# torchkge-team/torchkge

Measured on AMD Instinct MI355X. Metric: link-prediction triples scored/sec (filtered LP eval, both sides), higher is better.
Workload: dtype f32 (f16 hi/lo-split MFMA prefilter + exact f32 recheck; ranks bit-identical to f32)

## Files before the change

### torchkge_amd/csrc/kge_common.h

```cpp
#pragma once
#include <hip/hip_runtime.h>
#include <stdint.h>
#include <stdlib.h>
#include "../../include/kge_hip.h"

#define KGE_WAVE 64

#define KGE_CHECK_LAUNCH()                          \
    do {                                            \
        hipError_t e__ = hipGetLastError();         \
        if (e__ != hipSuccess) return (int)e__;     \
    } while (0)

static inline hipStream_t kge_s(kge_stream_t s) { return reinterpret_cast<hipStream_t>(s); }

int kge_bilinear_score_fwd(int kind, const float *t0, const float *t1, int d_ent, int d_rel, const int64_t *h,
                           const int64_t *t, const int64_t *r, int64_t B, float *out, hipStream_t s);
int kge_bilinear_score_bwd(int kind, const float *t0, const float *t1, int d_ent, int d_rel, const int64_t *h,
                           const int64_t *t, const int64_t *r, int64_t B, const float *go, float *g0, float *g1,
                           float *rows, int64_t rows_ld, hipStream_t s);

int kge_transr_score_fwd(const float *E, const float *R, const float *M, int d_ent, int d_rel, const int64_t *h,
                         const int64_t *t, const int64_t *r, int64_t B, float *out, hipStream_t s);
int kge_transr_score_bwd(const float *E, const float *R, const float *M, int d_ent, int d_rel, const int64_t *h,
                         const int64_t *t, const int64_t *r, int64_t B, const float *go, float *rows, int64_t rows_ld,
                         hipStream_t s);

static inline bool kge_aligned16(const void *p) { return (reinterpret_cast<uintptr_t>(p) & 15) == 0; }

__device__ __forceinline__ void kge_atomic_max_u32(unsigned *addr, unsigned v)
{
    if (v > __builtin_nontemporal_load(addr)) atomicMax(addr, v);
}

__device__ __forceinline__ float wave_sum(float v)
{
#pragma unroll
    for (int o = 32; o > 0; o >>= 1) v += __shfl_xor(v, o, 64);
    return v;
}
__device__ __forceinline__ int wave_sum_i(int v)
{
#pragma unroll
    for (int o = 32; o > 0; o >>= 1) v += __shfl_xor(v, o, 64);
    return v;
}

__device__ __forceinline__ float lp_chain_dot(const float *__restrict__ a, const float *__restrict__ t,
                                              int K, float acc)
{
    int kb = 0;
    for (; kb + 8 <= K; kb += 8) {
        float av[8], tv[8];
#pragma unroll
        for (int j = 0; j < 8; ++j) { av[j] = a[kb + j]; tv[j] = t[kb + j]; }
#pragma unroll
        for (int j = 0; j < 4; ++j) {
            acc = fmaf(av[j], tv[j], acc);
            acc = fmaf(av[4 + j], tv[4 + j], acc);
        }
    }
    if (kb < K) {
#pragma unroll
        for (int j = 0; j < 4; ++j) {
            const int k0 = kb + j, k1 = kb + 4 + j;
            if (k0 < K) acc = fmaf(a[k0], t[k0], acc);
            if (k1 < K) acc = fmaf(a[k1], t[k1], acc);
        }
    }
    return acc;
}

__device__ __forceinline__ float lp_epilogue(int mode, float dot, float qn, float en)
{
    if (mode == KGE_LP_L2_EXPAND) {
        float d2 = fmaf(-2.0f, dot, qn + en);
        return -fmaxf(d2, 0.0f);
    }
    return dot;
}

__device__ __forceinline__ float lp_epilogue_proj(int mode, float v0, float x, float y, float p, float z)
{
    float v;
    if (mode == KGE_LP_L2_PROJH) v = fmaf(x, fmaf(x, z, p), v0);
    else v = fmaf(y, fmaf(y, z, fmaf(2.0f, x, p)), v0);
    return -fmaxf(v, 0.0f);
}
__device__ __forceinline__ float lp_epilogue_any(const kge_lp_desc &d, float dot, int64_t i, int64_t c)
{
    if (d.mode == KGE_LP_DOT) return dot;
    const float v0 = fmaf(-2.0f, dot, d.qn[i] + d.en[c]);
    if (d.mode == KGE_LP_L2_EXPAND) return -fmaxf(v0, 0.0f);
    const float x = d.scal[d.r_idx[i] * d.scal_ld + c];
    const float y = d.mode == KGE_LP_L2_PROJD ? d.yc[c] : 0.f;
    return lp_epilogue_proj(d.mode, v0, x, y, d.Wq[i * d.ldw], d.Wq[i * d.ldw + 1]);
}

constexpr float KGE_TWO_PI_F = 6.2831855f;
template <int MODE>
__device__ __forceinline__ float lp_direct_term(float x)
{
    if (MODE == KGE_LP_TORUS_L1) {
        const float a = fabsf(x);
        return fminf(a, 1.0f - a);
    } else if (MODE == KGE_LP_TORUS_L2) {
        const float v = x * x;
        return fminf(v, 1.0f - v);
    } else if (MODE == KGE_LP_TORUS_EL2) {
        const float u = fminf(x, 1.0f - x);
        return 1.0f - cosf(KGE_TWO_PI_F * u);
    }
    return fabsf(x);
}
template <int MODE>
__device__ __forceinline__ float lp_direct_finish(float acc)
{
    if (MODE == KGE_LP_TORUS_L1) return -(2.0f * acc);
    if (MODE == KGE_LP_TORUS_L2) return -(4.0f * acc);
    if (MODE == KGE_LP_TORUS_EL2) return -(0.5f * acc);
    return -acc;
}
template <int MODE>
__device__ __forceinline__ float lp_group_chain(const float *q, const float *t, int K)
{
    float acc = 0.0f;
    for (int k = 0; k < K; k += 4) {
        float m[4];
#pragma unroll
        for (int e = 0; e < 4; ++e) m[e] = lp_direct_term<MODE>(k + e < K ? q[k + e] - t[k + e] : 0.0f);
        acc = acc + ((m[0] + m[1]) + (m[2] + m[3]));
    }
    return acc;
}

__device__ __forceinline__ float lp_pair_score(const kge_lp_desc &d, int64_t i, int64_t c)
{
    if (KGE_LP_IS_MFMA(d.mode)) {
        float acc = lp_chain_dot(d.A0 + i * d.lda0, d.T0 + c * d.ldt0, d.K0, 0.0f);
        if (d.K1 > 0) acc = lp_chain_dot(d.A1 + i * d.lda1, d.T1 + c * d.ldt1, d.K1, acc);
        return lp_epilogue_any(d, acc, i, c);
    }
    const float *q = d.A0 + i * d.lda0;
    const float *t = d.T0 + c * d.ldt0;
    switch (d.mode) {
    case KGE_LP_TORUS_L1: return lp_direct_finish<KGE_LP_TORUS_L1>(lp_group_chain<KGE_LP_TORUS_L1>(q, t, d.K0));
    case KGE_LP_TORUS_L2: return lp_direct_finish<KGE_LP_TORUS_L2>(lp_group_chain<KGE_LP_TORUS_L2>(q, t, d.K0));
    case KGE_LP_TORUS_EL2: return lp_direct_finish<KGE_LP_TORUS_EL2>(lp_group_chain<KGE_LP_TORUS_EL2>(q, t, d.K0));
    default: break;
    }
    float acc = 0.0f;
    const bool l1 = d.mode == KGE_LP_L1_DIRECT;
    const float a = d.Wq ? d.scal[c * d.scal_ld + (d.scal_ld > 1 ? d.r_idx[i] : 0)] : 0.0f;
    const float *w = d.Wq ? d.Wq + i * d.ldw : nullptr;
    if (l1) {
        for (int k = 0; k < d.K0; k += 4) {
            float m[4];
#pragma unroll
            for (int e = 0; e < 4; ++e) {
                float diff = 0.0f;
                if (k + e < d.K0) {
                    diff = q[k + e] - t[k + e];
                    if (w) diff = fmaf(a, w[k + e], diff);
                }
                m[e] = fabsf(diff);
            }
            acc = acc + ((m[0] + m[1]) + (m[2] + m[3]));
        }
    } else {
        for (int k = 0; k < d.K0; ++k) {
            float diff = q[k] - t[k];
            if (w) diff = fmaf(a, w[k], diff);
            acc = fmaf(diff, diff, acc);
        }
    }
    return -acc;
}

#ifndef KGE_PS_KC_V
#define KGE_PS_KC_V 32
#define KGE_PS_LD_V 36
#endif
constexpr int KGE_PS_KC = KGE_PS_KC_V, KGE_PS_LD = KGE_PS_LD_V;

static inline bool kge_lp_vec4(const kge_lp_desc &d)
{
    bool v = (d.K0 % 4 == 0) && (d.lda0 % 4 == 0) && (d.ldt0 % 4 == 0) && kge_aligned16(d.A0) && kge_aligned16(d.T0);
    if (d.K1 > 0)
        v = v && (d.K1 % 4 == 0) && (d.lda1 % 4 == 0) && (d.ldt1 % 4 == 0) && kge_aligned16(d.A1) && kge_aligned16(d.T1);
    return v;
}

template <int CH>
__device__ __forceinline__ float lp_chain_direct(const float *__restrict__ a, const float *__restrict__ t, int K, float acc)
{
    if (CH != 2) {
        constexpr int OP = CH == 1 ? (int)KGE_LP_L1_DIRECT : CH;
        for (int k = 0; k < K; k += 4) {
            const float4 av = *reinterpret_cast<const float4 *>(a + k), tv = *reinterpret_cast<const float4 *>(t + k);
            acc = acc + ((lp_direct_term<OP>(av.x - tv.x) + lp_direct_term<OP>(av.y - tv.y)) +
                         (lp_direct_term<OP>(av.z - tv.z) + lp_direct_term<OP>(av.w - tv.w)));
        }
    } else {
        for (int k = 0; k < K; ++k) {
            const float diff = a[k] - t[k];
            acc = fmaf(diff, diff, acc);
        }
    }
    return acc;
}

template <bool VEC4, int CH = 0>
__device__ __forceinline__ float lp_staged_segment(const float *__restrict__ A, int64_t lda,
                                                   const float *__restrict__ T, int64_t ldt, int K, int qi, int ci,
                                                   float *qs, float *es, float acc)
{
    const int lane = threadIdx.x & 63;
    static_assert(KGE_PS_KC == 32, "the fetch / store macros below are written out for 8 float4 pieces per row");
    int k0 = 0;
    if (VEC4 && K >= KGE_PS_KC) {
        float4 q0, q1, q2, q3, q4, q5, q6, q7, e0, e1, e2, e3, e4, e5, e6, e7;
#define KGE_PS_FETCH(IT, KK)                                                                                  \
    {                                                                                                         \
        const int idx_ = lane + 64 * IT, rr_ = idx_ >> 3, pc_ = idx_ & 7;                                     \
        const int rq_ = __shfl(qi, rr_, 64), rc_ = __shfl(ci, rr_, 64);                                      \
        q##IT = *reinterpret_cast<const float4 *>(A + (int64_t)rq_ * lda + (KK) + pc_ * 4);                   \
        e##IT = *reinterpret_cast<const float4 *>(T + (int64_t)rc_ * ldt + (KK) + pc_ * 4);                   \
    }
#define KGE_PS_STORE(IT)                                                                                      \
    {                                                                                                         \
        const int idx_ = lane + 64 * IT, rr_ = idx_ >> 3, pc_ = idx_ & 7;                                     \
        *reinterpret_cast<float4 *>(qs + rr_ * KGE_PS_LD + pc_ * 4) = q##IT;                                  \
        *reinterpret_cast<float4 *>(es + rr_ * KGE_PS_LD + pc_ * 4) = e##IT;                                  \
    }
#define KGE_PS_ALL(M, ...) M(0, ##__VA_ARGS__) M(1, ##__VA_ARGS__) M(2, ##__VA_ARGS__) M(3, ##__VA_ARGS__) \
                           M(4, ##__VA_ARGS__) M(5, ##__VA_ARGS__) M(6, ##__VA_ARGS__) M(7, ##__VA_ARGS__)
        KGE_PS_ALL(KGE_PS_FETCH, 0)
        for (; k0 + KGE_PS_KC <= K; k0 += KGE_PS_KC) {
            KGE_PS_ALL(KGE_PS_STORE)
            if (k0 + 2 * KGE_PS_KC <= K) { KGE_PS_ALL(KGE_PS_FETCH, k0 + KGE_PS_KC) }
            __builtin_amdgcn_fence(__ATOMIC_SEQ_CST, "wavefront");
            if (CH == 0) acc = lp_chain_dot(qs + lane * KGE_PS_LD, es + lane * KGE_PS_LD, KGE_PS_KC, acc);
            else acc = lp_chain_direct<CH>(qs + lane * KGE_PS_LD, es + lane * KGE_PS_LD, KGE_PS_KC, acc);
            __builtin_amdgcn_fence(__ATOMIC_SEQ_CST, "wavefront");
        }
#undef KGE_PS_ALL
#undef KGE_PS_STORE
#undef KGE_PS_FETCH
    }
// ... 120 lines not shown
```

### torchkge_amd/csrc/lp_split_mfma.hip

```cpp
#include "kge_common.h"
#ifndef KGE_BUILD_NO_SLP
#error "build with -fno-slp-vectorize -DKGE_BUILD_NO_SLP=1 (torchkge_amd/csrc/build.py): SLP-packed v_pk_fma_f32 with a lane-crossing op_sel misreads beside co-executing MFMAs (profiles/r06/slp_bisect.txt)"
#endif

typedef _Float16 f16x8 __attribute__((ext_vector_type(8)));
typedef float f32x2 __attribute__((ext_vector_type(2)));
typedef float f32x16 __attribute__((ext_vector_type(16)));

namespace {

constexpr int TQ = 192, TC = 256;
constexpr int NT = 3;
constexpr int E_STAGE_BYTES = TC * 128;
constexpr int Q_STAGE_BYTES = TQ * 128;
constexpr int STAGE_BYTES = E_STAGE_BYTES + Q_STAGE_BYTES;
constexpr int UNC_CAP = 2048;
constexpr int GSETS = 4;
constexpr int SMEM_BYTES = 2 * STAGE_BYTES + 16 + UNC_CAP * 4 + TQ * 20 + TQ * GSETS * 12 + 16;
constexpr int SPLIT_SCALE_LOG2 = 12;

struct SplitParams {
    const char *Es, *Qs;
    int row_bytes;
    int units;
// ... 1861 lines not shown
                            *p.overflow = 1.0f;
                        }
                    }
                    if (lane == 0) *unc_cnt = 0;
                }
            }
            if (GS && more && !(dbg & 16)) {
                if (LV == 1) { KGE_HLOAD(ah0, bh0, sb_next, 0) } else { KGE_SLOAD(ah0, al0, bh0, bl0, sb_next, 0) }
            }
            if (more) {
                int qp_next, ct_next;
                item_qp_ct(it + 1, qp_next, ct_next);
                const int64_t next_q0 = (int64_t)qp_next * TQ;
                if (next_q0 != cur_q0) {
                    flush_counts(cur_q0);
                    cur_q0 = next_q0;
                    load_panel(cur_q0);
                }
            }
        }
        if (DBG && tl) {
            tsv[15] = __builtin_readcyclecounter();
            if (lane == 0) {
                unsigned long long *o = reinterpret_cast<unsigned long long *>(p.list) + ((wid >> 2) * KGE_TL_STAGES + g) * 16;
#pragma unroll
                for (int i = 0; i < 16; ++i) o[i] = tsv[i];
            }
        }
        if (++s == S) { s = 0; ++it; }
    }
#undef KGE_TS
#undef KGE_SMMA_PA
#undef KGE_SMMA_P
#undef KGE_HLOAD
#undef KGE_HWAIT
#undef KGE_SLOAD
#undef KGE_SWAIT
#undef KGE_DSR
    flush_counts(cur_q0);
}

template <bool VEC4>
__global__ __launch_bounds__(64, 2) void split_recheck_kernel(const kge_lp_desc d, const float *__restrict__ s_true,
                                                           const int32_t *__restrict__ list, int32_t cap,
                                                           const int32_t *__restrict__ list_count, int32_t *raw_count,
                                                           float *list_stat)
{
    __shared__ __attribute__((aligned(16))) float qs[64 * KGE_PS_LD];
    __shared__ __attribute__((aligned(16))) float es[64 * KGE_PS_LD];
    const int lane = threadIdx.x;
    const int n = (int)min((unsigned)*list_count, (unsigned)cap);
    if (list_stat && blockIdx.x == 0 && lane == 0) atomicAdd(list_stat, (float)n);
    const int ngroups = (n + 63) >> 6;
    for (int grp = blockIdx.x; grp < ngroups; grp += gridDim.x) {
        const int pi = grp * 64 + lane;
        const bool valid = pi < n;
        const int pj = valid ? pi : grp * 64;
        const int qi = list[2 * pj], ci = list[2 * pj + 1];
        const float sc = lp_pair_score_staged<VEC4>(d, qi, ci, qs, es);
        if (valid && !(sc >= s_true[qi])) atomicSub(&raw_count[qi], 1);
    }
}

__device__ __forceinline__ float recheck_e_segment(const float *__restrict__ T, int64_t ldt, int K, int ci,
                                                   const float *__restrict__ qrow, float *es, float acc)
{
    const int lane = threadIdx.x & 63;
    int k0 = 0;
    if (K >= KGE_PS_KC) {
        float4 e0, e1, e2, e3, e4, e5, e6, e7;
#define KGE_RR_FETCH(IT, KK)                                                                                  \
    {                                                                                                         \
        const int idx_ = lane + 64 * IT, rr_ = idx_ >> 3, pc_ = idx_ & 7;                                     \
        const int rc_ = __shfl(ci, rr_, 64);                                                                  \
        e##IT = *reinterpret_cast<const float4 *>(T + (int64_t)rc_ * ldt + (KK) + pc_ * 4);                   \
    }
#define KGE_RR_STORE(IT)                                                                                      \
    {                                                                                                         \
        const int idx_ = lane + 64 * IT, rr_ = idx_ >> 3, pc_ = idx_ & 7;                                     \
        *reinterpret_cast<float4 *>(es + rr_ * KGE_PS_LD + pc_ * 4) = e##IT;                                  \
    }
#define KGE_RR_ALL(M, ...) M(0, ##__VA_ARGS__) M(1, ##__VA_ARGS__) M(2, ##__VA_ARGS__) M(3, ##__VA_ARGS__) \
                           M(4, ##__VA_ARGS__) M(5, ##__VA_ARGS__) M(6, ##__VA_ARGS__) M(7, ##__VA_ARGS__)
        KGE_RR_ALL(KGE_RR_FETCH, 0)
        for (; k0 + KGE_PS_KC <= K; k0 += KGE_PS_KC) {
            KGE_RR_ALL(KGE_RR_STORE)
            if (k0 + 2 * KGE_PS_KC <= K) { KGE_RR_ALL(KGE_RR_FETCH, k0 + KGE_PS_KC) }
            __builtin_amdgcn_fence(__ATOMIC_SEQ_CST, "wavefront");
            acc = lp_chain_dot(qrow + k0, es + lane * KGE_PS_LD, KGE_PS_KC, acc);
            __builtin_amdgcn_fence(__ATOMIC_SEQ_CST, "wavefront");
        }
#undef KGE_RR_ALL
#undef KGE_RR_STORE
#undef KGE_RR_FETCH
    }
    for (; k0 < K; k0 += KGE_PS_KC) {
        const int kc = min(KGE_PS_KC, K - k0);
        const int pieces = kc >> 2;
        for (int idx = lane; idx < 64 * pieces; idx += 64) {
            const int rr = idx / pieces, pc = idx - rr * pieces;
            const int rc = __shfl(ci, rr, 64);
            *reinterpret_cast<float4 *>(es + rr * KGE_PS_LD + pc * 4) =
                *reinterpret_cast<const float4 *>(T + (int64_t)rc * ldt + k0 + pc * 4);
        }
        __builtin_amdgcn_fence(__ATOMIC_SEQ_CST, "wavefront");
        acc = lp_chain_dot(qrow + k0, es + lane * KGE_PS_LD, kc, acc);
        __builtin_amdgcn_fence(__ATOMIC_SEQ_CST, "wavefront");
    }
    return acc;
}

constexpr int RR_ROWS = 32, RR_PANEL = 96;

constexpr int RR_G = 4;

template <int NWV>
__global__ __launch_bounds__(64 * NWV) void split_recheck_regions_kernel(const kge_lp_desc d, const float *__restrict__ s_true,
                                                                        const int32_t *__restrict__ list, int32_t region_cap,
                                                                        const int32_t *__restrict__ region_count, int n_regions,
                                                                        int ldq, int seg_cols, int32_t *raw_count, float *list_stat,
                                                                        int32_t *list_count)
{
    extern __shared__ __attribute__((aligned(16))) float rr_smem[];
    const int tid = threadIdx.x, lane = tid & 63, wv = tid >> 6;
    float *qrows = rr_smem;
    float *es = rr_smem + RR_ROWS * ldq + wv * 64 * KGE_PS_LD;
    const int K = d.K0 + d.K1;
    int n_block = 0;
    auto stage = [&](int64_t q0, int c0, int c1) {
        const int np = (c1 - c0) >> 2;
        for (int idx = tid; idx < RR_ROWS * np; idx += 64 * NWV) {
            const int rr = idx / np, pc = idx - rr * np;
            const int64_t q = min(q0 + rr, d.B - 1);
            const int col = c0 + pc * 4;
            const float4 v = col < d.K0 ? *reinterpret_cast<const float4 *>(d.A0 + q * d.lda0 + col)
                                        : *reinterpret_cast<const float4 *>(d.A1 + q * d.lda1 + (col - d.K0));
            *reinterpret_cast<float4 *>(qrows + rr * ldq + pc * 4) = v;
        }
    };
    auto chain = [&](float acc, int ci, const float *qrow, int c0, int c1) -> float {
        if (c0 < d.K0) acc = recheck_e_segment(d.T0 + c0, d.ldt0, min(c1, d.K0) - c0, ci, qrow, es, acc);
        if (c1 > d.K0 && d.K1 > 0) {
            const int s0 = max(c0, d.K0);
            acc = recheck_e_segment(d.T1 + (s0 - d.K0), d.ldt1, c1 - s0, ci, qrow + (s0 - c0), es, acc);
        }
        return acc;
    };
    for (int reg = blockIdx.x; reg < n_regions; reg += gridDim.x) {
        const int n = (int)min((unsigned)region_count[reg], (unsigned)region_cap);
        if (n == 0) continue;
        n_block += n;
        const int64_t q0 = (int64_t)(reg / 3) * RR_PANEL + (reg % 3) * RR_ROWS;
        const int2 *ent = reinterpret_cast<const int2 *>(list) + (int64_t)reg * region_cap;
        if (K <= seg_cols) {
            __syncthreads();
            stage(q0, 0, K);
            __syncthreads();
            for (int c0 = wv * 64; c0 < n; c0 += NWV * 64) {
                const int pi = c0 + lane;
                const bool valid = pi < n;
                const int2 e = ent[valid ? pi : c0];
                const int qi = e.x, ci = e.y;
                const float acc = chain(0.0f, ci, qrows + (int)(qi - q0) * ldq, 0, K);
                const float sc = lp_epilogue_any(d, acc, qi, ci);
                if (valid && !(sc >= s_true[qi])) atomicSub(&raw_count[qi], 1);
            }
            continue;
        }
        for (int b0 = 0; b0 < n; b0 += NWV * 64 * RR_G) {
            float acc[RR_G];
            int qi[RR_G], ci[RR_G];
#pragma unroll
            for (int g = 0; g < RR_G; ++g) {
                const int c0 = b0 + (g * NWV + wv) * 64;
                const int pi = c0 + lane;
                const int2 e = ent[min(pi < n ? pi : c0, n - 1)];
                qi[g] = e.x; ci[g] = e.y; acc[g] = 0.0f;
            }
            for (int c0 = 0; c0 < K; c0 += seg_cols) {
                const int c1 = min(K, c0 + seg_cols);
                __syncthreads();
                stage(q0, c0, c1);
                __syncthreads();
#pragma unroll
                for (int g = 0; g < RR_G; ++g)
                    if (b0 + (g * NWV + wv) * 64 < n)
                        acc[g] = chain(acc[g], ci[g], qrows + (int)(qi[g] - q0) * ldq, c0, c1);
            }
#pragma unroll
            for (int g = 0; g < RR_G; ++g) {
                const int pi = b0 + (g * NWV + wv) * 64 + lane;
                if (pi < n) {
                    const float sc = lp_epilogue_any(d, acc[g], qi[g], ci[g]);
                    if (!(sc >= s_true[qi[g]])) atomicSub(&raw_count[qi[g]], 1);
                }
            }
        }
    }
    if (tid == 0 && n_block > 0) {
        if (list_stat) atomicAdd(list_stat, (float)n_block);
        if (list_count) atomicAdd(list_count, n_block);
    }
}

template <int NWAVES, bool DBG, int PM, int GS = 0, int LV = 0>
int launch_split(const SplitParams &p, int grid, hipStream_t s)
{
    auto k = lp_split_count_kernel<NWAVES, DBG, PM, GS, LV>;
    static int attr_dev[16];
    if (int e = kge_ensure_dyn_smem(reinterpret_cast<const void *>(k), SMEM_BYTES, attr_dev)) return e;
    hipLaunchKernelGGL(k, dim3(grid), dim3(64 * NWAVES), SMEM_BYTES, s, p);
    KGE_CHECK_LAUNCH();
    return 0;
}

int split_num_cus()
{
    static int n = 0;
    if (n == 0) {
        int dev = 0;
        hipDeviceProp_t prop;
        if (hipGetDevice(&dev) == hipSuccess && hipGetDeviceProperties(&prop, dev) == hipSuccess)
            n = prop.multiProcessorCount;
        if (n <= 0) n = 256;
    }
    return n;
}

inline int64_t round_up(int64_t x, int64_t m) { return (x + m - 1) / m * m; }

}

extern "C" int kge_lp_split_units(int K, int with_aug)
{
    return (int)round_up((K + (with_aug ? 1 : 0) + 15) / 16, 2);
}

extern "C" int64_t kge_lp_split_rows_padded(int64_t rows, int is_query) { return round_up(rows, is_query ? TQ : TC); }

extern "C" int kge_lp_split_rows(const float *X0, int64_t ld0, int K0, const float *X1, int64_t ld1, int K1,
                                 int64_t rows, int is_query, int aug_mode, const float *aug, float aug_mul,
                                 const float *norm2max0, const float *norm2max1, void *out, float *cell_ss,
                                 const int64_t *row_index, kge_stream_t stream)
{
    if (rows < 0 || K0 <= 0 || K1 < 0 || ld0 < K0 || (K1 > 0 && ld1 < K1) || aug_mode < 0 || aug_mode > 4)
        return KGE_EINVAL;
    if (rows == 0 && is_query) return 0;
    if ((rows > 0 && !X0) || (rows > 0 && K1 > 0 && !X1) || !out || ((aug_mode == 1 || aug_mode == 3) && rows > 0 && !aug))
        return KGE_EINVAL;
    SplitRowsParams p;
    p.X0 = X0; p.X1 = X1; p.ld0 = ld0; p.ld1 = ld1; p.K0 = K0; p.K1 = K1;
    p.rows = rows;
    p.rows_p = kge_lp_split_rows_padded(rows, is_query);
    p.aug_mode = aug_mode; p.aug = aug; p.aug_mul = aug_mul;
    p.nmax0 = norm2max0; p.nmax1 = norm2max1;
    p.units_p = kge_lp_split_units(K0 + K1, aug_mode != 0);
    p.out = reinterpret_cast<uint4 *>(out);
    p.cell_ss = cell_ss;
    p.row_index = row_index;
    const int64_t total = (p.rows_p / 16) * ((p.units_p + 15) / 16);
    if (total == 0) return 0;
    const int grid = (int)(total < 65536 ? total : 65536);
    hipLaunchKernelGGL(split_rows_kernel, dim3(grid), dim3(256), 0, kge_s(stream), p);
    KGE_CHECK_LAUNCH();
    return 0;
}

extern "C" int kge_lp_hi_units(int K) { return (int)round_up((K + 2 + 15) / 16, 4); }

static int hi_rows_impl(const float *X0, int64_t ld0, int K0, const float *X1, int64_t ld1, int K1, int64_t rows,
                        int is_query, int aug_mode, const float *aug, float aug_mul, const float *norm2max0,
                        const float *norm2max1, void *out, float *dn2, float *dn2max, const int64_t *row_index,
                        int frag, kge_stream_t stream)
{
    if (rows < 0 || K0 <= 0 || K1 < 0 || ld0 < K0 || (K1 > 0 && ld1 < K1) || aug_mode < 1 || aug_mode > 4) return KGE_EINVAL;
    if (rows == 0 && is_query) return 0;
    if ((rows > 0 && !X0) || (rows > 0 && K1 > 0 && !X1) || !out || ((aug_mode == 1 || aug_mode == 3) && rows > 0 && !aug))
        return KGE_EINVAL;
    HiRowsParams p;
    p.X0 = X0; p.X1 = X1; p.ld0 = ld0; p.ld1 = ld1; p.K0 = K0; p.K1 = K1;
    p.rows = rows;
    p.rows_p = kge_lp_split_rows_padded(rows, is_query);
    p.aug_mode = aug_mode; p.aug = aug; p.aug_mul = aug_mul;
    p.nmax0 = norm2max0; p.nmax1 = norm2max1;
    p.units_p = kge_lp_hi_units(K0 + K1);
    p.out = reinterpret_cast<uint4 *>(out);
    p.dn2 = dn2; p.dn2max = dn2max; p.row_index = row_index;
    p.frag = frag;
    p.nm_bmax = nullptr; p.nm_blocks = 0; p.dn_bmax = nullptr; p.prev_nmax = nullptr; p.nm_out = nullptr;
    const int64_t blocks = p.rows_p / 16;
    if (blocks == 0) return 0;
    const int64_t cap = dn2max ? 2 * (int64_t)split_num_cus() : 65536;
    hipLaunchKernelGGL(hi_rows_kernel, dim3((int)(blocks < cap ? blocks : cap)), dim3(256), 0, kge_s(stream), p);
    KGE_CHECK_LAUNCH();
    return 0;
}

extern "C" int kge_lp_hi_rows(const float *X0, int64_t ld0, int K0, const float *X1, int64_t ld1, int K1, int64_t rows,
                              int is_query, int aug_mode, const float *aug, float aug_mul, const float *norm2max0,
                              const float *norm2max1, void *out, float *dn2, float *dn2max, const int64_t *row_index,
                              kge_stream_t stream)
{
    return hi_rows_impl(X0, ld0, K0, X1, ld1, K1, rows, is_query, aug_mode, aug, aug_mul, norm2max0, norm2max1, out, dn2,
                        dn2max, row_index, 0, stream);
}

extern "C" int kge_lp_hi_rows_frag(const float *X0, int64_t ld0, int K0, const float *X1, int64_t ld1, int K1, int64_t rows,
                                   int aug_mode, const float *aug, float aug_mul, const float *norm2max0,
                                   const float *norm2max1, void *out, float *dn2, float *dn2max, kge_stream_t stream)
{
    return hi_rows_impl(X0, ld0, K0, X1, ld1, K1, rows, 0, aug_mode, aug, aug_mul, norm2max0, norm2max1, out, dn2, dn2max,
                        nullptr, 1, stream);
}

extern "C" int kge_lp_dot_table_prep_blocks(int64_t rows, int which)
{
    if (which == 0) { const int64_t b = (rows + 63) / 64; return (int)(b < 2048 ? (b > 0 ? b : 1) : 2048); }
    const int64_t b = kge_lp_split_rows_padded(rows, 0) / 16;
    return (int)(b < 4096 ? (b > 0 ? b : 1) : 4096);
}

extern "C" int kge_lp_dot_table_prep(const float *X0, int64_t ld0, int K0, const float *X1, int64_t ld1, int K1, int64_t rows,
                                     int frag, float *norm2max0_io, float *norm2max1_io, void *out, float *dn_block_max,
                                     float *ws, kge_stream_t stream)
{
    if (rows <= 0 || K0 <= 0 || K1 < 0 || ld0 < K0 || (K1 > 0 && ld1 < K1)) return KGE_EINVAL;
    if (!X0 || (K1 > 0 && (!X1 || !norm2max1_io)) || !norm2max0_io || !out || !dn_block_max || !ws) return KGE_EINVAL;
    const int nb = kge_lp_dot_table_prep_blocks(rows, 0);
    hipLaunchKernelGGL(dot_table_norm_max_kernel, dim3(nb), dim3(256), 0, kge_s(stream), X0, ld0, K0,
                       K1 > 0 ? X1 : nullptr, ld1, K1, rows, ws);
    KGE_CHECK_LAUNCH();
    HiRowsParams p;
    p.X0 = X0; p.X1 = K1 > 0 ? X1 : nullptr; p.ld0 = ld0; p.ld1 = ld1; p.K0 = K0; p.K1 = K1;
    p.rows = rows;
    p.rows_p = kge_lp_split_rows_padded(rows, 0);
    p.aug_mode = 4; p.aug = nullptr; p.aug_mul = 0.f;
    p.nmax0 = norm2max0_io; p.nmax1 = K1 > 0 ? norm2max1_io : nullptr;
    p.units_p = kge_lp_hi_units(K0 + K1);
    p.out = reinterpret_cast<uint4 *>(out);
    p.dn2 = nullptr; p.dn2max = nullptr; p.row_index = nullptr;
    p.frag = frag ? 1 : 0;
    p.nm_bmax = ws; p.nm_blocks = nb; p.dn_bmax = dn_block_max; p.prev_nmax = nullptr; p.nm_out = nullptr;
    static const int old_only = getenv("KGE_HIROWS_OLD") ? atoi(getenv("KGE_HIROWS_OLD")) : 0;
    const bool vec = K0 % 4 == 0 && K1 % 4 == 0 && ld0 % 4 == 0 && ((size_t)X0 & 15) == 0 &&
                     (K1 == 0 || (ld1 % 4 == 0 && ((size_t)X1 & 15) == 0));
    if (frag && vec && !old_only)
        hipLaunchKernelGGL(hi_rows_frag_kernel<false>, dim3(kge_lp_dot_table_prep_blocks(rows, 1)), dim3(256), 0, kge_s(stream), p);
    else
        hipLaunchKernelGGL(hi_rows_kernel, dim3(kge_lp_dot_table_prep_blocks(rows, 1)), dim3(256), 0, kge_s(stream), p);
    KGE_CHECK_LAUNCH();
    return 0;
// ... 135 lines not shown
    p.dbg = kge_env_int("KGE_SPLIT_DBG", 0);
    p.qg = kge_env_int("KGE_SPLIT_QG", (int64_t)TQ * p.row_bytes * 16 <= (3 << 20) ? 16 : 4);
    const int slots = split_num_cus();
    if (a->es_frag) {
        const bool chunked = units > kge_hi_stream_max_units() ||
                             (kge_env_int("KGE_HC_FORCE", 0) && kge_hi_chunk_supported(units) && !a->members && !a->region_count &&
                              d->mode < KGE_LP_L2_PROJH);
        const bool grouped = a->members && a->n_multi_p > 0;
        if (!lv1 || (chunked && !kge_hi_chunk_supported(units))) return KGE_EINVAL;
        if ((a->members != nullptr) != (a->n_multi_p > 0) || (grouped && (chunked || proj || a->region_count || !a->col_q)))
            return KGE_EINVAL;
        if (grouped && (a->n_multi_p % TQ || GSETS != 4)) return KGE_EINVAL;
        kge_hi_stream_params h;
        h.Ef = reinterpret_cast<const char *>(Es);
        h.Qh = reinterpret_cast<const char *>(Qs);
        h.q_row_bytes = p.row_bytes;
        h.units = units; h.units_p = units_p;
        h.rows_p = kge_lp_split_rows_padded(d->N, 0);
        h.q_rows = a->col_q ? a->n_single_p : Bp;
        if (a->col_q && (a->n_single_p <= 0 || a->n_single_p % TQ)) return KGE_EINVAL;
        h.B = d->B;
        h.thr = p.thr; h.thr4 = p.thr4;
        h.X = p.X; h.ldx = p.ldx; h.r_idx = p.r_idx; h.yc = p.yc;
        h.raw_count = raw_count; h.list = list; h.cap = cap; h.list_count = list_count; h.overflow = overflow;
        h.col_q = a->col_q;
        h.members = nullptr;
        h.region_count = nullptr; h.region_cap = 0;
        if (a->region_count) {
            if (a->col_q || !kge_lp_split_regions_supported(d)) return KGE_EINVAL;
            const int n_regions = kge_lp_split_regions(d->B);
            h.region_count = a->region_count;
            h.region_cap = cap / n_regions;
            if (h.region_cap <= 0) return KGE_EINVAL;
        }
        h.true_idx = a->true_idx; h.c_base = d->c_base;
        const int pm = d->mode == KGE_LP_L2_PROJH ? 1 : (d->mode == KGE_LP_L2_PROJD ? 2 : 0);
        if (chunked) {
            if (pm != 0 || h.region_count) return KGE_EUNSUPPORTED;
            return kge_hi_chunk_launch(h, slots, s);
        }
        if (!grouped) return kge_hi_stream_launch(h, pm, slots, s);
        if (a->n_single_p > 0) {
            rc = kge_hi_stream_launch(h, pm, slots, s);
            if (rc) return rc;
        }
        h.Qh = reinterpret_cast<const char *>(Qs) + a->n_single_p * (int64_t)p.row_bytes;
        h.q_rows = a->n_multi_p;
        h.col_q = nullptr;
        h.members = a->members;
        return kge_hi_stream_launch(h, 0, slots, s);
    }
    if (a->col_q || a->members) {
        if (a->n_single_p < 0 || a->n_multi_p < 0 || a->n_single_p % TQ || a->n_multi_p % TQ ||
            (a->n_single_p > 0 && !a->col_q) || (a->n_multi_p > 0 && !a->members))
            return KGE_EINVAL;
        const int pm = d->mode == KGE_LP_L2_PROJH ? 1 : (d->mode == KGE_LP_L2_PROJD ? 2 : 0);
        if (a->n_single_p > 0) {
            p.col_q = a->col_q;
            p.q_panels = (int)(a->n_single_p / TQ);
            p.n_items = (int64_t)p.q_panels * p.c_tiles;
            const int grid = (int)(p.n_items < slots ? p.n_items : slots);
            rc = lv1 ? (pm == 1 ? launch_split<8, false, 1, 0, 1>(p, grid, s)
                                : (pm == 2 ? launch_split<8, false, 2, 0, 1>(p, grid, s) : launch_split<8, false, 0, 0, 1>(p, grid, s)))
                     : (pm == 1 ? launch_split<8, false, 1>(p, grid, s)
                                : (pm == 2 ? launch_split<8, false, 2>(p, grid, s) : launch_split<8, false, 0>(p, grid, s)));
            if (rc) return rc;
        }
        if (a->n_multi_p > 0) {
            p.col_q = nullptr;
            p.members = a->members;
            p.Qs = reinterpret_cast<const char *>(Qs) + a->n_single_p * (int64_t)p.row_bytes;
            p.q_panels = (int)(a->n_multi_p / TQ);
            p.n_items = (int64_t)p.q_panels * p.c_tiles;
            const int grid = (int)(p.n_items < slots ? p.n_items : slots);
            rc = lv1 ? (pm == 1 ? launch_split<8, false, 1, GSETS, 1>(p, grid, s)
                                : (pm == 2 ? launch_split<8, false, 2, GSETS, 1>(p, grid, s) : launch_split<8, false, 0, GSETS, 1>(p, grid, s)))
                     : (pm == 1 ? launch_split<8, false, 1, GSETS>(p, grid, s)
                                : (pm == 2 ? launch_split<8, false, 2, GSETS>(p, grid, s) : launch_split<8, false, 0, GSETS>(p, grid, s)));
        }
        return rc;
    }
    p.q_panels = (int)((d->B + TQ - 1) / TQ);
    p.n_items = (int64_t)p.q_panels * p.c_tiles;
    const int grid = (int)(p.n_items < slots ? p.n_items : slots);
    if (lv1 && d->mode == KGE_LP_L2_PROJH) return launch_split<8, false, 1, 0, 1>(p, grid, s);
    if (lv1 && d->mode == KGE_LP_L2_PROJD) return launch_split<8, false, 2, 0, 1>(p, grid, s);
    if (lv1) return p.dbg ? launch_split<8, true, 0, 0, 1>(p, grid, s) : launch_split<8, false, 0, 0, 1>(p, grid, s);
    if (d->mode == KGE_LP_L2_PROJH) return launch_split<8, false, 1>(p, grid, s);
    if (d->mode == KGE_LP_L2_PROJD) return launch_split<8, false, 2>(p, grid, s);
    return p.dbg ? launch_split<8, true, 0>(p, grid, s) : launch_split<8, false, 0>(p, grid, s);
}

extern "C" int kge_lp_split_group_sets(void) { return GSETS; }

extern "C" int kge_lp_split_recheck(const kge_lp_desc *d, const float *s_true, const int32_t *list, int32_t cap,
                                    const int32_t *list_count, int32_t *raw_count, float *list_stat, kge_stream_t stream)
{
    int rc = kge_lp_desc_check(d);
    if (rc) return rc;
    if (d->B == 0 || d->N == 0) return 0;
    if (!s_true || !list || cap <= 0 || !list_count || !raw_count) return KGE_EINVAL;
    if (!KGE_LP_IS_MFMA(d->mode)) return KGE_EINVAL;
    const bool vec4 = kge_lp_vec4(*d);
    const int grid = split_num_cus() * kge_env_int("KGE_SPLIT_RECHECK_WAVES", 160 * 1024 / (2 * 64 * KGE_PS_LD * 4));
    if (vec4)
        hipLaunchKernelGGL(split_recheck_kernel<true>, dim3(grid), dim3(64), 0, kge_s(stream), *d, s_true, list, cap,
                           list_count, raw_count, list_stat);
    else
        hipLaunchKernelGGL(split_recheck_kernel<false>, dim3(grid), dim3(64), 0, kge_s(stream), *d, s_true, list,
                           cap, list_count, raw_count, list_stat);
    KGE_CHECK_LAUNCH();
    return 0;
}

extern "C" int kge_lp_split_regions(int64_t B)
{
    return (int)(kge_lp_split_rows_padded(B, 1) / RR_PANEL) * 3;
}

static int region_seg_cols(int K)
{
    const int max_ld = kge_env_int("KGE_REGION_MAX_BYTES", 36 * 1024) / (RR_ROWS * 4);
    const int ld_full = K + (((K >> 2) & 1) ? 0 : 4);
    if (ld_full <= max_ld) return K;
    const int seg_ld = min(max_ld, kge_env_int("KGE_REGION_SEG_BYTES", 20 * 1024) / (RR_ROWS * 4));
    int seg = ((seg_ld - 4) / 32) * 32;
    return seg < 32 ? 32 : seg;
}

extern "C" int kge_lp_split_regions_supported(const kge_lp_desc *d)
{
    if (kge_lp_desc_check(d) || !KGE_LP_IS_MFMA(d->mode) || !kge_lp_vec4(*d)) return 0;
    const int K = d->K0 + d->K1;
    if ((K + 2 + 15) / 16 > 32) return 0;
    if (region_seg_cols(K) < K && kge_env_int("KGE_REGION_SEGMENTS", 1) == 0) return 0;
    return 1;
}

extern "C" int kge_lp_split_recheck_regions(const kge_lp_desc *d, const float *s_true, const int32_t *list, int32_t cap,
                                            const int32_t *region_count, int32_t *raw_count, float *list_stat,
                                            int32_t *list_count, kge_stream_t stream)
{
    int rc = kge_lp_desc_check(d);
    if (rc) return rc;
    if (d->B == 0 || d->N == 0) return 0;
    if (!s_true || !list || cap <= 0 || !region_count || !raw_count) return KGE_EINVAL;
    if (!kge_lp_split_regions_supported(d)) return KGE_EINVAL;
    const int n_regions = kge_lp_split_regions(d->B);
    const int32_t region_cap = cap / n_regions;
    if (region_cap <= 0) return KGE_EINVAL;
    const int K = d->K0 + d->K1;
    const int seg = region_seg_cols(K);
    const int ldq = seg + (((seg >> 2) & 1) ? 0 : 4);
    const int nwv = kge_env_int("KGE_RECHECK_REGION_WAVES", 2);
    const int smem = (RR_ROWS * ldq + (nwv == 4 ? 4 : 2) * 64 * KGE_PS_LD) * 4;
    const int want = split_num_cus() * 6;
    const int grid = n_regions < want ? n_regions : want;
    static int attr2[16], attr4[16];
    if (nwv == 4) {
        auto k = split_recheck_regions_kernel<4>;
        if (int e = kge_ensure_dyn_smem(reinterpret_cast<const void *>(k), smem, attr4)) return e;
        hipLaunchKernelGGL(k, dim3(grid), dim3(256), smem, kge_s(stream), *d, s_true, list, region_cap, region_count, n_regions,
                           ldq, seg, raw_count, list_stat, list_count);
    } else {
        auto k = split_recheck_regions_kernel<2>;
        if (int e = kge_ensure_dyn_smem(reinterpret_cast<const void *>(k), smem, attr2)) return e;
        hipLaunchKernelGGL(k, dim3(grid), dim3(128), smem, kge_s(stream), *d, s_true, list, region_cap, region_count, n_regions,
                           ldq, seg, raw_count, list_stat, list_count);
    }
    KGE_CHECK_LAUNCH();
    return 0;
}

extern "C" int kge_absmax(const float *x, int64_t n, float *max_io, kge_stream_t stream)
{
    if (n < 0 || !max_io) return KGE_EINVAL;
    if (n == 0) return 0;
    if (!x) return KGE_EINVAL;
    const int64_t want = (n + 1023) / 1024;
    const int grid = (int)(want < 1024 ? want : 1024);
    hipLaunchKernelGGL(absmax_kernel, dim3(grid), dim3(256), 0, kge_s(stream), x, n, max_io);
    KGE_CHECK_LAUNCH();
    return 0;
}


extern "C" int kge_mfma_f16_selftest(void)
{
    constexpr int NT_ = 8;
    float ab[NT_][32], c[NT_], expect[NT_];
    for (int t = 0; t < NT_; ++t) { for (int k = 0; k < 32; ++k) ab[t][k] = 0.f; c[t] = 0.f; }
    auto A = [&](int t, int k) -> float & { return ab[t][k]; };
    auto Bv = [&](int t, int k) -> float & { return ab[t][16 + k]; };
    for (int k = 0; k < 16; ++k) { A(0, k) = 1.f; Bv(0, k) = 1.f; } A(0, 0) = 4096.f; Bv(0, 0) = 4096.f; expect[0] = 16777232.f;
    A(1, 0) = A(1, 1) = A(1, 2) = 1.f; Bv(1, 0) = Bv(1, 1) = Bv(1, 2) = 1.f; c[1] = 16777216.f; expect[1] = 16777220.f;
    A(2, 0) = 1.f; Bv(2, 0) = 1.f; c[2] = 16777216.f; expect[2] = 16777216.f;
    for (int k = 0; k < 16; ++k) { A(3, k) = 1.f; Bv(3, k) = 1.f; } A(3, 0) = 4096.f; Bv(3, 0) = 4096.f; A(3, 1) = 4096.f; Bv(3, 1) = -4096.f; expect[3] = 14.f;
    for (int k = 0; k < 16; ++k) { A(4, k) = 0.5f; Bv(4, k) = 1.f; } A(4, 0) = 4096.f; Bv(4, 0) = 4096.f; A(4, 1) = 4096.f; Bv(4, 1) = -4096.f; expect[4] = 4.f;
    A(5, 0) = 4096.f; Bv(5, 0) = 4096.f; A(5, 1) = 1.f; Bv(5, 1) = 1.f; A(5, 2) = 0.5f; Bv(5, 2) = 1.f; expect[5] = 16777216.f;
    A(6, 0) = 1.f; Bv(6, 0) = 1.f; A(6, 8) = 0.5f; Bv(6, 8) = 1.f; c[6] = 16777216.f; expect[6] = 16777216.f;
    A(7, 0) = 9.5367431640625e-07f; Bv(7, 0) = 1024.f; expect[7] = 0.0009765625f;
    float *d_ab = nullptr, *d_c = nullptr, *d_out = nullptr, got[NT_];
    hipError_t e = hipMalloc(&d_ab, sizeof(ab));
    if (e == hipSuccess) e = hipMalloc(&d_c, sizeof(c));
    if (e == hipSuccess) e = hipMalloc(&d_out, sizeof(got));
    if (e == hipSuccess) e = hipMemcpy(d_ab, ab, sizeof(ab), hipMemcpyHostToDevice);
    if (e == hipSuccess) e = hipMemcpy(d_c, c, sizeof(c), hipMemcpyHostToDevice);
    if (e == hipSuccess) {
        hipLaunchKernelGGL(mfma_selftest_kernel, dim3(1), dim3(64), 0, 0, d_ab, d_c, d_out, NT_);
        e = hipGetLastError();
    }
    if (e == hipSuccess) e = hipMemcpy(got, d_out, sizeof(got), hipMemcpyDeviceToHost);
    if (d_ab) (void)hipFree(d_ab);
    if (d_c) (void)hipFree(d_c);
    if (d_out) (void)hipFree(d_out);
    if (e != hipSuccess) return (int)e;
    for (int t = 0; t < NT_; ++t)
        if (got[t] != expect[t]) return 0;
    return 1;
}

extern "C" int kge_lp_dot_table_prep_fused(const float *X0, int64_t ld0, int K0, const float *X1, int64_t ld1, int K1,
                                           int64_t rows, const float *prev_nmax, void *out, float *dn_block_max,
                                           float *nm_block_max, kge_stream_t stream)
{
    if (rows <= 0 || K0 <= 0 || K1 < 0 || ld0 < K0 || (K1 > 0 && ld1 < K1)) return KGE_EINVAL;
    if (!X0 || (K1 > 0 && !X1) || !prev_nmax || !out || !dn_block_max || !nm_block_max) return KGE_EINVAL;
    const bool vec = K0 % 4 == 0 && K1 % 4 == 0 && ld0 % 4 == 0 && ((size_t)X0 & 15) == 0 &&
                     (K1 == 0 || (ld1 % 4 == 0 && ((size_t)X1 & 15) == 0));
    if (!vec) return KGE_EINVAL;
    HiRowsParams p;
    p.X0 = X0; p.X1 = K1 > 0 ? X1 : nullptr; p.ld0 = ld0; p.ld1 = ld1; p.K0 = K0; p.K1 = K1;
    p.rows = rows;
    p.rows_p = kge_lp_split_rows_padded(rows, 0);
    p.aug_mode = 4; p.aug = nullptr; p.aug_mul = 0.f;
    p.nmax0 = nullptr; p.nmax1 = nullptr;
    p.units_p = kge_lp_hi_units(K0 + K1);
    p.out = reinterpret_cast<uint4 *>(out);
    p.dn2 = nullptr; p.dn2max = nullptr; p.row_index = nullptr;
    p.frag = 1;
    p.nm_bmax = nullptr; p.nm_blocks = 0; p.dn_bmax = dn_block_max; p.prev_nmax = prev_nmax; p.nm_out = nm_block_max;
    hipLaunchKernelGGL(hi_rows_frag_kernel<true>, dim3(kge_lp_dot_table_prep_blocks(rows, 1)), dim3(256), 0, kge_s(stream), p);
    KGE_CHECK_LAUNCH();
    return 0;
}

extern "C" int kge_lp_dot_query_pipeline(int side, const float *E0, const float *E1, const float *R0, const float *R1, int d,
                                         const int64_t *h, const int64_t *t, const int64_t *r, int64_t B,
                                         const float *emax0, const float *emax1, const float *de2max, float *qmax_io,
                                         int accum_model, float eps_scale, float *Q0, float *Q1, float *qn, float *s_true,
                                         void *Qh, float *thr, float *q_dn2, int32_t *list_count, float *overflow,
                                         int32_t *zero_i32, int64_t zero_n, const float *dn_block_max, int dn_blocks,
                                         const float *nm_block_max, int nm_blocks, float *prev_nmax, kge_stream_t stream)
{
    if (dn_block_max && dn_blocks <= 0) return KGE_EINVAL;
    if (nm_block_max && nm_blocks <= 0) return KGE_EINVAL;
    const bool both = side == KGE_SIDE_BOTH, cplx = E1 != nullptr;
    if ((side != KGE_SIDE_TAIL && side != KGE_SIDE_HEAD && !both) || d <= 0 || d > 4096 || B < 0) return KGE_EINVAL;
    if (B == 0) return 0;
    if (!E0 || !R0 || !h || !t || !r || !emax0 || !de2max || !Q0 || !qn || !s_true || !Qh || !thr || !list_count || !overflow)
        return KGE_EINVAL;
    if (cplx && (!R1 || !Q1 || !emax1)) return KGE_EINVAL;
    if (!cplx && (R1 || Q1)) return KGE_EINVAL;
    if (d % 8 != 0 || !kge_aligned16(E0) || !kge_aligned16(R0) || (cplx && (!kge_aligned16(E1) || !kge_aligned16(R1))))
        return KGE_EINVAL;
    if (zero_n < 0 || (zero_n > 0 && !zero_i32)) return KGE_EINVAL;
    DotPipeParams p;
    p.tail = both ? 2 : (side == KGE_SIDE_TAIL ? 1 : 0);
    p.Bh = B;
    p.E0 = E0; p.E1 = E1; p.R0 = R0; p.R1 = R1; p.d = d; p.h = h; p.t = t; p.r = r;
    p.B = both ? 2 * B : B; p.Bp = kge_lp_split_rows_padded(p.B, 1);
    p.emax0 = emax0; p.emax1 = cplx ? emax1 : nullptr; p.de2max = de2max; p.qmax_io = qmax_io;
    p.c_acc = accum_model == 1 ? 1.25f : 2.0f; p.eps_scale = eps_scale;
    const int K = cplx ? 2 * d : d;
    p.units = (K + 2 + 15) / 16; p.units_p = kge_lp_hi_units(K);
    p.Q0 = Q0; p.Q1 = Q1; p.qn = qn; p.s_true = s_true; p.q_dn2 = q_dn2;
    p.thr = reinterpret_cast<float2 *>(thr);
    p.Qh = reinterpret_cast<_Float16 *>(Qh);
    p.list_count = list_count; p.overflow = overflow;
    p.zero_i32 = zero_i32; p.zero_n = zero_n;
    p.dn_bmax = dn_block_max; p.dn_blocks = dn_blocks;
    p.nm_bmax = nm_block_max; p.nm_blocks = nm_blocks; p.prev_nmax = prev_nmax;
    const int qpw = kge_env_int("KGE_DQPIPE_QPW", p.Bp / 16 < 2048 ? 4 : 16);
    const int64_t groups = (p.Bp + qpw - 1) / qpw, blocks = (groups + 3) / 4;
    const int grid = (int)(blocks < 256 * 16 ? blocks : 256 * 16);
    if (qpw == 4) {
        if (cplx) hipLaunchKernelGGL((dot_query_pipeline_kernel<4, true>), dim3(grid), dim3(256), 0, kge_s(stream), p);
        else hipLaunchKernelGGL((dot_query_pipeline_kernel<4, false>), dim3(grid), dim3(256), 0, kge_s(stream), p);
    } else {
        if (cplx) hipLaunchKernelGGL((dot_query_pipeline_kernel<16, true>), dim3(grid), dim3(256), 0, kge_s(stream), p);
        else hipLaunchKernelGGL((dot_query_pipeline_kernel<16, false>), dim3(grid), dim3(256), 0, kge_s(stream), p);
    }
    KGE_CHECK_LAUNCH();
    return 0;
}

extern "C" int kge_lp_query_pipeline(int side, const float *E, const float *R, int d, const int64_t *h,
                                     const int64_t *t, const int64_t *r, int64_t B, const float *en,
                                     const float *emax, float *qmax_io, int accum_model, float eps_scale, float *Q,
                                     float *qn, float *s_true, void *Qs, float *thr, int32_t *list_count,
                                     const float *e2pref, const int32_t *qs_row, int level, const float *de2max,
                                     float *q_dn2, const float *tp_block_max, int tp_blocks, int32_t *zero_i32,
                                     int64_t zero_n, kge_stream_t stream)
{
    if (level != 0 && level != 1) return KGE_EINVAL;
    if (level == 1 && !de2max) return KGE_EINVAL;
    const bool both = side == KGE_SIDE_BOTH;
    if ((side != KGE_SIDE_TAIL && side != KGE_SIDE_HEAD && !both) || d <= 0 || d > 4096 || B < 0) return KGE_EINVAL;
    if (B == 0) return 0;
    if (!E || !R || !h || !t || !r || !en || !emax || !Q || !qn || !s_true || !Qs || !thr || !list_count) return KGE_EINVAL;
// ... 33 lines not shown
```

Baseline: 1370 billion.

## Add row-staged recheck kernel with prefetched entity rows for small K

Adds a new recheck kernel for the case where K fits in one segment. Each wave handles P candidates per pass: it cooperatively fetches the entity rows into registers one pass ahead, then stores them to LDS and computes the f32 dot from LDS rows, with the epilogue terms also prefetched. The old in-kernel small-K path in the region recheck kernel is removed and replaced by dispatch to this kernel. The aim is to hide gather latency and replace strided per-lane global row reads with coalesced loads. The cost is heavy register use from up to 36 named float4s, and only 16 of 64 lanes doing dot-product work.

```diff
diff --git a/torchkge_amd/csrc/kge_common.h b/torchkge_amd/csrc/kge_common.h
--- a/torchkge_amd/csrc/kge_common.h
+++ b/torchkge_amd/csrc/kge_common.h
@@ -95,6 +95,61 @@
     const float x = d.scal[d.r_idx[i] * d.scal_ld + c];
     const float y = d.mode == KGE_LP_L2_PROJD ? d.yc[c] : 0.f;
     return lp_epilogue_proj(d.mode, v0, x, y, d.Wq[i * d.ldw], d.Wq[i * d.ldw + 1]);
+}
+
+struct lp_epi_terms { float qn, en, x, y, p, z; };
+__device__ __forceinline__ lp_epi_terms lp_epilogue_terms(const kge_lp_desc &d, int64_t i, int64_t c)
+{
+    lp_epi_terms t = {0.f, 0.f, 0.f, 0.f, 0.f, 0.f};
+    if (d.mode == KGE_LP_DOT) return t;
+    t.qn = d.qn[i];
+    t.en = d.en[c];
+    if (d.mode == KGE_LP_L2_EXPAND) return t;
+    t.x = d.scal[d.r_idx[i] * d.scal_ld + c];
+    t.y = d.mode == KGE_LP_L2_PROJD ? d.yc[c] : 0.f;
+    t.p = d.Wq[i * d.ldw];
+    t.z = d.Wq[i * d.ldw + 1];
+    return t;
+}
+__device__ __forceinline__ float lp_epilogue_from_terms(const kge_lp_desc &d, float dot, const lp_epi_terms &t)
+{
+    if (d.mode == KGE_LP_DOT) return dot;
+    const float v0 = fmaf(-2.0f, dot, t.qn + t.en);
+    if (d.mode == KGE_LP_L2_EXPAND) return -fmaxf(v0, 0.0f);
+    return lp_epilogue_proj(d.mode, v0, t.x, t.y, t.p, t.z);
+}
+
+__device__ __forceinline__ float lp_chain_dot_rows(const float *__restrict__ a, const float *__restrict__ t, int K, float acc)
+{
+    const int K8 = K & ~7;
+    float4 a0[4], a1[4], t0[4], t1[4];
+#define KGE_CD_LOAD(S, KB)                                                                                    \
+    {                                                                                                         \
+        a0[S] = *reinterpret_cast<const float4 *>(a + (KB)); a1[S] = *reinterpret_cast<const float4 *>(a + (KB) + 4); \
+        t0[S] = *reinterpret_cast<const float4 *>(t + (KB)); t1[S] = *reinterpret_cast<const float4 *>(t + (KB) + 4); \
+    }
+#pragma unroll
+    for (int s = 0; s < 4; ++s)
+        if (8 * s < K8) KGE_CD_LOAD(s, 8 * s)
+    for (int kb = 0; kb < K8; kb += 32) {
+#pragma unroll
+        for (int s = 0; s < 4; ++s) {
+            if (kb + 8 * s < K8) {
+                acc = fmaf(a0[s].x, t0[s].x, acc); acc = fmaf(a1[s].x, t1[s].x, acc);
+                acc = fmaf(a0[s].y, t0[s].y, acc); acc = fmaf(a1[s].y, t1[s].y, acc);
+                acc = fmaf(a0[s].z, t0[s].z, acc); acc = fmaf(a1[s].z, t1[s].z, acc);
+                acc = fmaf(a0[s].w, t0[s].w, acc); acc = fmaf(a1[s].w, t1[s].w, acc);
+                if (kb + 32 + 8 * s < K8) KGE_CD_LOAD(s, kb + 32 + 8 * s)
+            }
+        }
+    }
+#undef KGE_CD_LOAD
+    if (K8 < K) {
+        const float4 av = *reinterpret_cast<const float4 *>(a + K8), tv = *reinterpret_cast<const float4 *>(t + K8);
+        acc = fmaf(av.x, tv.x, acc); acc = fmaf(av.y, tv.y, acc);
+        acc = fmaf(av.z, tv.z, acc); acc = fmaf(av.w, tv.w, acc);
+    }
+    return acc;
 }
 
 constexpr float KGE_TWO_PI_F = 6.2831855f;
diff --git a/torchkge_amd/csrc/lp_split_mfma.hip b/torchkge_amd/csrc/lp_split_mfma.hip
--- a/torchkge_amd/csrc/lp_split_mfma.hip
+++ b/torchkge_amd/csrc/lp_split_mfma.hip
@@ -2037,21 +2037,6 @@
         n_block += n;
         const int64_t q0 = (int64_t)(reg / 3) * RR_PANEL + (reg % 3) * RR_ROWS;
         const int2 *ent = reinterpret_cast<const int2 *>(list) + (int64_t)reg * region_cap;
-        if (K <= seg_cols) {
-            __syncthreads();
-            stage(q0, 0, K);
-            __syncthreads();
-            for (int c0 = wv * 64; c0 < n; c0 += NWV * 64) {
-                const int pi = c0 + lane;
-                const bool valid = pi < n;
-                const int2 e = ent[valid ? pi : c0];
-                const int qi = e.x, ci = e.y;
-                const float acc = chain(0.0f, ci, qrows + (int)(qi - q0) * ldq, 0, K);
-                const float sc = lp_epilogue_any(d, acc, qi, ci);
-                if (valid && !(sc >= s_true[qi])) atomicSub(&raw_count[qi], 1);
-            }
-            continue;
-        }
         for (int b0 = 0; b0 < n; b0 += NWV * 64 * RR_G) {
             float acc[RR_G];
             int qi[RR_G], ci[RR_G];
@@ -2082,6 +2067,124 @@
             }
         }
     }
+    if (tid == 0 && n_block > 0) {
+        if (list_stat) atomicAdd(list_stat, (float)n_block);
+        if (list_count) atomicAdd(list_count, n_block);
+    }
+}
+
+constexpr int RW_P = 16;
+constexpr int RW_MAX_PIECES = 72;
+
+template <int NWV, int P, int NIT>
+__global__ __launch_bounds__(64 * NWV) void split_recheck_rows_kernel(const kge_lp_desc d, const float *__restrict__ s_true,
+                                                                     const int32_t *__restrict__ list, int32_t region_cap,
+                                                                     const int32_t *__restrict__ region_count, int n_regions,
+                                                                     int ldq, int32_t *raw_count, float *list_stat,
+                                                                     int32_t *list_count)
+{
+    static_assert(P % 8 == 0 && P >= 8 && P <= 32 && NIT <= 9, "8 lanes fetch a row piece; the named row registers below");
+    constexpr int NH = P / 8;
+    extern __shared__ __attribute__((aligned(16))) float rr_smem[];
+    const int tid = threadIdx.x, lane = tid & 63, wv = tid >> 6;
+    float *qrows = rr_smem;
+    float *es = rr_smem + RR_ROWS * ldq + wv * P * ldq;
+    const int K = d.K0 + d.K1, np = K >> 2, np0 = d.K0 >> 2;
+    const int lr = lane >> 3, pc0 = lane & 7;
+    int n_block = 0;
+    for (int reg = blockIdx.x; reg < n_regions; reg += gridDim.x) {
+        const int n = (int)min((unsigned)region_count[reg], (unsigned)region_cap);
+        if (n == 0) continue;
+        n_block += n;
+        const int64_t q0 = (int64_t)(reg / 3) * RR_PANEL + (reg % 3) * RR_ROWS;
+        const int2 *ent = reinterpret_cast<const int2 *>(list) + (int64_t)reg * region_cap;
+        const int npass = (n + P - 1) / P;
+        auto entry = [&](int ps) -> int2 {
+            const int pi = ps * P + lane;
+            return ent[(lane < P && pi < n) ? pi : ps * P];
+        };
+        float4 ev00, ev01, ev02, ev03, ev04, ev05, ev06, ev07, ev08, ev10, ev11, ev12, ev13, ev14, ev15, ev16, ev17, ev18,
+               ev20, ev21, ev22, ev23, ev24, ev25, ev26, ev27, ev28, ev30, ev31, ev32, ev33, ev34, ev35, ev36, ev37, ev38;
+#define KGE_RW_ITS(M, H) M(H, 0) M(H, 1) M(H, 2) M(H, 3) M(H, 4) M(H, 5) M(H, 6) M(H, 7) M(H, 8)
+#define KGE_RW_FETCH_IT(H, IT)                                                                                \
+    if constexpr (H < NH && IT < NIT) {                                                                       \
+        const int pc_ = pc0 + 8 * IT;                                                                         \
+        if (8 * IT < np && rowok_ && pc_ < np)                                                                \
+            ev##H##IT = *reinterpret_cast<const float4 *>((pc_ < np0 ? b0_ : b1_) + pc_ * 4);                 \
+    }
+#define KGE_RW_FETCH_H(H, E, PS)                                                                              \
+    if constexpr (H < NH) {                                                                                   \
+        const int row_ = H * 8 + lr;                                                                          \
+        const int rc_ = __shfl((E).y, row_, 64);                                                              \
+        const float *b0_ = d.T0 + (int64_t)rc_ * d.ldt0;                                                      \
+        const float *b1_ = d.K1 > 0 ? d.T1 + (int64_t)rc_ * d.ldt1 - d.K0 : b0_;                              \
+        const bool rowok_ = (PS) * P + row_ < n;                                                              \
+        KGE_RW_ITS(KGE_RW_FETCH_IT, H)                                                                        \
+    }
+#define KGE_RW_FETCH(E, PS) { KGE_RW_FETCH_H(0, E, PS) KGE_RW_FETCH_H(1, E, PS) KGE_RW_FETCH_H(2, E, PS) KGE_RW_FETCH_H(3, E, PS) }
+#define KGE_RW_STORE_IT(H, IT)                                                                                \
+    if constexpr (H < NH && IT < NIT) {                                                                       \
+        const int pc_ = pc0 + 8 * IT;                                                                         \
+        if (8 * IT < np && rowok_ && pc_ < np) *reinterpret_cast<float4 *>(es + row_ * ldq + pc_ * 4) = ev##H##IT; \
+    }
+#define KGE_RW_STORE_H(H, PS)                                                                                 \
+    if constexpr (H < NH) {                                                                                   \
+        const int row_ = H * 8 + lr;                                                                          \
+        const bool rowok_ = (PS) * P + row_ < n;                                                              \
+        KGE_RW_ITS(KGE_RW_STORE_IT, H)                                                                        \
+    }
+#define KGE_RW_STORE(PS) { KGE_RW_STORE_H(0, PS) KGE_RW_STORE_H(1, PS) KGE_RW_STORE_H(2, PS) KGE_RW_STORE_H(3, PS) }
+        int ps = wv;
+        int2 e1 = make_int2(0, 0), e2 = make_int2(0, 0);
+        lp_epi_terms t1 = {0.f, 0.f, 0.f, 0.f, 0.f, 0.f};
+        float st1 = 0.f;
+        if (ps < npass) {
+            e1 = entry(ps);
+            t1 = lp_epilogue_terms(d, e1.x, e1.y);
+            st1 = s_true[e1.x];
+            KGE_RW_FETCH(e1, ps)
+            e2 = entry(min(ps + NWV, npass - 1));
+        }
+        __syncthreads();
+        for (int idx = tid; idx < RR_ROWS * np; idx += 64 * NWV) {
+            const int rr = idx / np, pc = idx - rr * np;
+            const int64_t q = min(q0 + rr, d.B - 1);
+            const int col = pc * 4;
+            const float4 v = col < d.K0 ? *reinterpret_cast<const float4 *>(d.A0 + q * d.lda0 + col)
+                                        : *reinterpret_cast<const float4 *>(d.A1 + q * d.lda1 + (col - d.K0));
+            *reinterpret_cast<float4 *>(qrows + rr * ldq + pc * 4) = v;
+        }
+        __syncthreads();
+        for (; ps < npass; ps += NWV) {
+            KGE_RW_STORE(ps)
+            const int2 e0 = e1;
+            const lp_epi_terms t0 = t1;
+            const float st0 = st1;
+            if (ps + NWV < npass) {
+                e1 = e2;
+                t1 = lp_epilogue_terms(d, e1.x, e1.y);
+                st1 = s_true[e1.x];
+                KGE_RW_FETCH(e1, ps + NWV)
+            }
+            e2 = entry(min(ps + 2 * NWV, npass - 1));
+            __builtin_amdgcn_fence(__ATOMIC_SEQ_CST, "wavefront");
+            if (lane < P && ps * P + lane < n) {
+                const float *qrow = qrows + (int)(e0.x - q0) * ldq, *erow = es + lane * ldq;
+                float acc = lp_chain_dot_rows(qrow, erow, d.K0, 0.0f);
+                if (d.K1 > 0) acc = lp_chain_dot_rows(qrow + d.K0, erow + d.K0, d.K1, acc);
+                const float sc = lp_epilogue_from_terms(d, acc, t0);
+                if (!(sc >= st0)) atomicSub(&raw_count[e0.x], 1);
+            }
+            __builtin_amdgcn_fence(__ATOMIC_SEQ_CST, "wavefront");
+        }
+    }
+#undef KGE_RW_STORE
+#undef KGE_RW_STORE_H
+#undef KGE_RW_STORE_IT
+#undef KGE_RW_FETCH
+#undef KGE_RW_FETCH_H
+#undef KGE_RW_FETCH_IT
+#undef KGE_RW_ITS
     if (tid == 0 && n_block > 0) {
         if (list_stat) atomicAdd(list_stat, (float)n_block);
         if (list_count) atomicAdd(list_count, n_block);
@@ -2523,10 +2626,27 @@
     const int K = d->K0 + d->K1;
     const int seg = region_seg_cols(K);
     const int ldq = seg + (((seg >> 2) & 1) ? 0 : 4);
+    const int want = split_num_cus() * 6;
+    const int grid = n_regions < want ? n_regions : want;
+    if (K <= seg && (K >> 2) <= RW_MAX_PIECES) {
+        const int smem = (RR_ROWS + 2 * RW_P) * ldq * 4;
+        static int attr_s[16], attr_l[16];
+        if (K <= 32 * 7) {
+            auto k = split_recheck_rows_kernel<2, RW_P, 7>;
+            if (int e = kge_ensure_dyn_smem(reinterpret_cast<const void *>(k), smem, attr_s)) return e;
+            hipLaunchKernelGGL(k, dim3(grid), dim3(128), smem, kge_s(stream), *d, s_true, list, region_cap, region_count,
+                               n_regions, ldq, raw_count, list_stat, list_count);
+        } else {
+            auto k = split_recheck_rows_kernel<2, RW_P, RW_MAX_PIECES / 8>;
+            if (int e = kge_ensure_dyn_smem(reinterpret_cast<const void *>(k), smem, attr_l)) return e;
+            hipLaunchKernelGGL(k, dim3(grid), dim3(128), smem, kge_s(stream), *d, s_true, list, region_cap, region_count,
+                               n_regions, ldq, raw_count, list_stat, list_count);
+        }
+        KGE_CHECK_LAUNCH();
+        return 0;
+    }
     const int nwv = kge_env_int("KGE_RECHECK_REGION_WAVES", 2);
     const int smem = (RR_ROWS * ldq + (nwv == 4 ? 4 : 2) * 64 * KGE_PS_LD) * 4;
-    const int want = split_num_cus() * 6;
-    const int grid = n_regions < want ? n_regions : want;
     static int attr2[16], attr4[16];
     if (nwv == 4) {
         auto k = split_recheck_regions_kernel<4>;
```

New measurement: 1075 billion. 21.6% lower.
